# embedded-software-laboratory/p-dmpc

Hardware: AMD Instinct MI355X
Metric: MPC steps/sec (whole node) + p50 per-step plan latency, N vehicles H=8 (higher is better)
Workload: dtype f64

## Files before the change

include/pdmpc.h:

```cpp
#ifndef PDMPC_H
#define PDMPC_H

#include <stddef.h>
#include <stdint.h>

#ifdef __cplusplus
extern "C" {
#endif

#define PDMPC_HP_MAX 16
#define PDMPC_VMAX 8
#define PDMPC_JOINT_MAX 4

enum {
    PDMPC_OK = 0,
    PDMPC_EXHAUSTED = 1,
    PDMPC_ARENA_OVERFLOW = 2,
    PDMPC_ERR_INVALID = -1,
    PDMPC_ERR_NO_DEVICE = -2,
    PDMPC_ERR_HIP = -3,
    PDMPC_ERR_CAPACITY = -4,
    PDMPC_ERR_NO_MPA = -5
};

// ... 54 lines not shown
    const double* right_y;
    pdmpc_polygon_set obstacles;
    pdmpc_polygon_set dynamic_obstacles;
    pdmpc_polygon_set hdv_reachable_sets;
} pdmpc_vehicle_in;

typedef struct {
    int32_t status;
    int32_t n_expanded;
    int32_t n_popped;
    int32_t n_hp;
    int32_t tree_path[PDMPC_HP_MAX + 1];
    int32_t predicted_trims[PDMPC_HP_MAX];
    int32_t shape_cols[PDMPC_HP_MAX];
    int32_t _pad;
    double y_predicted[PDMPC_HP_MAX][3];
    double shapes[PDMPC_HP_MAX][2][PDMPC_VMAX];
    double path_nodes[PDMPC_HP_MAX + 1][8];
} pdmpc_vehicle_out;

typedef struct {
    int64_t n_vehicles;
    int64_t nodes_popped;
    int64_t nodes_generated;
    int64_t obstacle_columns;
    int64_t algorithmic_bytes;
    double kernel_ms;
    int64_t lds_bytes;
    int64_t lds_nodes;
    int64_t n_launches;
    int64_t queue_fallbacks;
    int64_t speculation_arrivals;
    int64_t edge_checks;
    int64_t segment_pair_tests;
    int64_t kernel;
    int64_t nodes_processed;
    int64_t rounds;
    int64_t shared_rounds;
    int64_t helper_checked;
    int64_t safe_replans;
    int64_t bad_status_plans;
} pdmpc_stats;


int pdmpc_create(const pdmpc_config* config, pdmpc_handle** out_handle);
int pdmpc_destroy(pdmpc_handle* handle);

int pdmpc_get_config(pdmpc_handle* handle, pdmpc_config* config, int32_t* mpa_uploaded);

int pdmpc_upload_mpa(pdmpc_handle* handle, const pdmpc_mpa* mpa);
int pdmpc_mpa_reach_host(const pdmpc_mpa* mpa, double* dmax, double* amax);
int pdmpc_reach_lists_host(int32_t Hp, double dmax, double amax, double root_x, double root_y, const double* x, const double* y, const int32_t* step_first,
                           const int32_t* step_count, int32_t* list_offset, int32_t* list);

int pdmpc_plan_batch(pdmpc_handle* handle, int32_t n_vehicles, const pdmpc_vehicle_in* in,
                     pdmpc_vehicle_out* out);

int pdmpc_set_arena_limit(pdmpc_handle* handle, int32_t max_nodes_limit);
int pdmpc_grow_arena(pdmpc_handle* handle, int32_t max_nodes);
int pdmpc_arena_nodes(pdmpc_handle* handle, int32_t* max_nodes, int64_t* regrows);

int pdmpc_plan_step(pdmpc_handle* handle, int32_t n_vehicles, const pdmpc_vehicle_in* in, const int32_t* pred_offset,
                    const int32_t* pred_index, const pdmpc_polygon_set* fallback_shapes, pdmpc_vehicle_out* out);

int pdmpc_plan_step_literal(pdmpc_handle* handle, int32_t n_vehicles, const pdmpc_vehicle_in* in, const int32_t* pred_offset, const int32_t* pred_index,
                            const pdmpc_polygon_set* fallback_shapes, pdmpc_vehicle_out* out);

int pdmpc_pack_batch(pdmpc_handle* handle, int32_t n_vehicles, const pdmpc_vehicle_in* in);
int pdmpc_plan_step_lean(pdmpc_handle* handle, int32_t n_vehicles, const pdmpc_vehicle_in* in, const int32_t* pred_offset, const int32_t* pred_index,
                         const pdmpc_polygon_set* fallback_shapes, int32_t* status, double* final_cost);
int pdmpc_fetch_records_at(pdmpc_handle* handle, int32_t count, const int32_t* vehicles, pdmpc_vehicle_out* out);
typedef struct {
    int32_t n_cells;
    int32_t n_graphs;
    int32_t n_picks;
    int32_t _pad;
    const int32_t* cell_offset;
    const int32_t* cell_slot;
    const int32_t* graph_offset;
    const int32_t* pick_graph;
    const int32_t* pick_offset;
    const int32_t* pick_slot;
} pdmpc_choice;
int pdmpc_choose_host(int32_t n, const int32_t* status, const double* final_cost, const pdmpc_choice* choice, int32_t* chosen, double* cell_cost);
int pdmpc_choose_resident(pdmpc_handle* handle, int32_t n, const pdmpc_choice* choice, int32_t* chosen, double* cell_cost, pdmpc_vehicle_out* picks);
int pdmpc_plan_step_chosen(pdmpc_handle* handle, int32_t n_vehicles, const pdmpc_vehicle_in* in, const int32_t* pred_offset, const int32_t* pred_index,
                           const pdmpc_polygon_set* fallback_shapes, const pdmpc_choice* choice, int32_t* chosen, double* cell_cost, pdmpc_vehicle_out* picks);
int pdmpc_choice_kernel_ms(pdmpc_handle* handle, double* ms);
int pdmpc_last_call_timing(pdmpc_handle* handle, double* us3);
int pdmpc_launch_packed(pdmpc_handle* handle);
int pdmpc_launch_range(pdmpc_handle* handle, int32_t first, int32_t count);
int pdmpc_fetch_results(pdmpc_handle* handle, int32_t n_vehicles, pdmpc_vehicle_out* out);
int pdmpc_synchronize(pdmpc_handle* handle);
int pdmpc_set_safe_launch(pdmpc_handle* handle, int32_t on);
int pdmpc_set_device_share(pdmpc_handle* handle, int32_t n_handles);
int pdmpc_begin_step(pdmpc_handle* handle);
int pdmpc_select_bank(pdmpc_handle* handle, int32_t bank);
int pdmpc_reset_stats(pdmpc_handle* handle);

int pdmpc_set_step_weights(pdmpc_handle* handle, int32_t n_vehicles, const double* weights);
int pdmpc_pack_step(pdmpc_handle* handle, int32_t n_vehicles, const pdmpc_vehicle_in* in,
                    const int32_t* pred_offset, const int32_t* pred_index,
                    const pdmpc_polygon_set* fallback_shapes);

int pdmpc_result_device_buffer(pdmpc_handle* handle, void** dev_ptr, size_t* nbytes);
int pdmpc_import_results(pdmpc_handle* handle, int32_t first, int32_t n, const void* dev_records);
// ... 223 lines not shown
```

include/pdmpc_reach.h:

```cpp
#ifndef PDMPC_REACH_H
#define PDMPC_REACH_H

#include <math.h>

#include "pdmpc_math.h"

#define PDMPC_REACH_FINITE 0x1p64
#define PDMPC_REACH_MARGIN 0x1p-20

PDMPC_HD static inline double pdmpc_reach_radius(double dmax, double amax, int k) {
    const double r = (double)(k - 1) * dmax + amax;
    return r + r * 0x1p-50;
}

PDMPC_HD static inline void pdmpc_reach_box(double dmax, double amax, int k, double root_x, double root_y, double* box) {
    const double R = pdmpc_reach_radius(dmax, amax, k);
    const double rho = R + PDMPC_REACH_MARGIN * (1.0 + fabs(root_x) + fabs(root_y) + R);
    box[0] = root_x - rho;
    box[1] = root_x + rho;
    box[2] = root_y - rho;
    box[3] = root_y + rho;
}

PDMPC_HD static inline int pdmpc_reach_in(double x0, double y0, double x1, double y1, double x_lo, double x_hi, double y_lo, double y_hi) {
    if (x0 != x0 || y0 != y0 || x1 != x1 || y1 != y1) return 0;
    const int bounded = fabs(x0) <= PDMPC_REACH_FINITE && fabs(y0) <= PDMPC_REACH_FINITE && fabs(x1) <= PDMPC_REACH_FINITE && fabs(y1) <= PDMPC_REACH_FINITE;
    if (!bounded) return 1;
    const double max_x = x0 > x1 ? x0 : x1, min_x = x0 < x1 ? x0 : x1;
    const double max_y = y0 > y1 ? y0 : y1, min_y = y0 < y1 ? y0 : y1;
    return !(max_x < x_lo || min_x > x_hi || max_y < y_lo || min_y > y_hi);
}

#endif
```

p-dmpc_amd/csrc/api.cpp:

```cpp
#include <hip/hip_runtime.h>

#include <algorithm>
#include <cmath>
#include <cstdio>
#include <cstdlib>
#include <chrono>
#include <cstring>
#include <limits>
#include <map>
#include <mutex>
#include <string>
#include <utility>
#include <vector>

#include "../../include/pdmpc_geometry.h"
#include "../../include/pdmpc_reach.h"
#include "handle.hpp"

namespace {

thread_local std::string g_err;

inline uint32_t align16(uint32_t v) { return (v + 15u) & ~15u; }

// ... 446 lines not shown
    }
    (void)hipMemsetAsync(h->d_flag.p, 0, h->d_flag.cap * sizeof(uint32_t), h->stream);
    (void)hipMemsetAsync(h->d_tree_size.p, 0, h->d_tree_size.cap * sizeof(int32_t), h->stream);
    (void)hipMemsetAsync(h->d_tie_count.p, 0, 4 * sizeof(int32_t), h->stream);
    (void)hipMemsetAsync(h->d_work_count.p, 0, 16 * sizeof(unsigned long long), h->stream);
    (void)hipMemsetAsync(h->d_out.p, 0, h->d_out.cap * sizeof(pdmpc_vehicle_out), h->stream);
    (void)hipStreamSynchronize(h->stream);
    *out_handle = h;
    return PDMPC_OK;
}

int pdmpc_destroy(pdmpc_handle* h) {
    if (!h) return PDMPC_OK;
    DeviceGuard device_guard__(h->cfg.device);
    delete h;
    return PDMPC_OK;
}

static void mpa_reach(const pdmpc_mpa* mpa, double& dmax, double& amax) {
    dmax = 0.0;
    amax = 0.0;
    for (int t = 0; t < mpa->n_maneuvers; ++t) {
        const pdmpc_maneuver& m = mpa->maneuvers[t];
        dmax = std::max(dmax, hypot(m.dx, m.dy));
        const double(*src[3])[PDMPC_VMAX] = {m.area, m.area_without_offset, m.area_large_offset};
        for (int a = 0; a < 3; ++a)
            for (int v = 0; v < m.n_cols && v < PDMPC_VMAX; ++v) amax = std::max(amax, hypot(src[a][0][v], src[a][1][v]));
    }
}

int pdmpc_mpa_reach_host(const pdmpc_mpa* mpa, double* dmax, double* amax) {
    if (!mpa || !dmax || !amax || (mpa->n_maneuvers > 0 && !mpa->maneuvers)) return fail(PDMPC_ERR_INVALID, "pdmpc_mpa_reach_host: null argument");
    mpa_reach(mpa, *dmax, *amax);
    return PDMPC_OK;
}

int pdmpc_reach_lists_host(int32_t Hp, double dmax, double amax, double root_x, double root_y, const double* x, const double* y, const int32_t* step_first,
                           const int32_t* step_count, int32_t* list_offset, int32_t* list) {
    if (Hp < 1 || Hp > PDMPC_HP_MAX || !step_first || !step_count || !list_offset) return fail(PDMPC_ERR_INVALID, "pdmpc_reach_lists_host: bad argument");
    int32_t n = 0;
    for (int k = 1; k <= Hp; ++k) {
        const int32_t a = step_first[k - 1], c = step_count[k - 1];
        if (a < 0 || c < 0 || (c > 1 && (!x || !y || !list))) return fail(PDMPC_ERR_INVALID, "pdmpc_reach_lists_host: bad step ranges");
        double box[4];
        pdmpc_reach_box(dmax, amax, k, root_x, root_y, box);
        list_offset[k - 1] = n;
        for (int32_t j = 0; j + 1 < c; ++j)
            if (pdmpc_reach_in(x[a + j], y[a + j], x[a + j + 1], y[a + j + 1], box[0], box[1], box[2], box[3])) list[n++] = j;
    }
    list_offset[Hp] = n;
    return PDMPC_OK;
}

int pdmpc_upload_mpa(pdmpc_handle* h, const pdmpc_mpa* mpa) {
    if (!h || !mpa) return fail(PDMPC_ERR_INVALID, "null argument");
    if (mpa->n_trims < 1 || mpa->n_trims > 1023) return fail(PDMPC_ERR_INVALID, "n_trims must be in 1..1023");
    if (mpa->Hp < h->cfg.Hp) return fail(PDMPC_ERR_INVALID, "mpa.Hp smaller than config.Hp");
    if (!mpa->transition || !mpa->maneuver_index || (mpa->n_maneuvers > 0 && !mpa->maneuvers)) return fail(PDMPC_ERR_INVALID, "null table");
    ON_DEVICE(h->cfg.device);
    const int n = mpa->n_trims, Hp = h->cfg.Hp;
    const int nw = (n + 63) / 64;
    std::vector<uint64_t> mask((size_t)Hp * n * nw + 2, 0);
    for (int k = 0; k < Hp; ++k)
        for (int i = 0; i < n; ++i)
            for (int j = 0; j < n; ++j)
                if (mpa->transition[((size_t)k * n + i) * n + j]) {
                    const int mi = mpa->maneuver_index[i * n + j];
                    if (mi < 0 || mi >= mpa->n_maneuvers) return fail(PDMPC_ERR_INVALID, "transition allowed but maneuver missing");
                    mask[((size_t)k * n + i) * nw + j / 64] |= 1ull << (j % 64);
                }
    std::vector<int16_t> mi((size_t)n * n + 8, -1);
    for (int i = 0; i < n * n; ++i) mi[i] = (int16_t)mpa->maneuver_index[i];
    const int T = mpa->n_maneuvers;
    std::vector<DevManPose> pose((size_t)std::max(T, 1));
    std::vector<double> area((size_t)std::max(T, 1) * 3 * PDMPC_VMAX * 2 + 2, 0.0);
    for (int t = 0; t < T; ++t) {
        const pdmpc_maneuver& m = mpa->maneuvers[t];
        if (m.n_cols < 2 || m.n_cols > PDMPC_VMAX) return fail(PDMPC_ERR_INVALID, "maneuver area column count out of range");
        pose[t].dx = m.dx;
        pose[t].dy = m.dy;
        pose[t].dyaw = m.dyaw;
        pose[t].n_cols = m.n_cols;
        pose[t].pad = 0;
        const double(*src[3])[PDMPC_VMAX] = {m.area, m.area_without_offset, m.area_large_offset};
        for (int a = 0; a < 3; ++a)
            for (int v = 0; v < m.n_cols; ++v) {
                area[(((size_t)t * 3 + a) * PDMPC_VMAX + v) * 2 + 0] = src[a][0][v];
                area[(((size_t)t * 3 + a) * PDMPC_VMAX + v) * 2 + 1] = src[a][1][v];
            }
    }
    mpa_reach(mpa, area[(size_t)T * 3 * PDMPC_VMAX * 2], area[(size_t)T * 3 * PDMPC_VMAX * 2 + 1]);
    if (h->d_mask.ensure(mask.size()) || h->d_mi.ensure(mi.size()) || h->d_pose.ensure(pose.size()) || h->d_area.ensure(area.size()))
        return fail(PDMPC_ERR_HIP, "hipMalloc failed for the MPA tables");
    HIPCHK(hipMemcpy(h->d_mask.p, mask.data(), mask.size() * 8, hipMemcpyHostToDevice));
    HIPCHK(hipMemcpy(h->d_mi.p, mi.data(), mi.size() * 2, hipMemcpyHostToDevice));
    HIPCHK(hipMemcpy(h->d_pose.p, pose.data(), pose.size() * sizeof(DevManPose), hipMemcpyHostToDevice));
    HIPCHK(hipMemcpy(h->d_area.p, area.data(), area.size() * 8, hipMemcpyHostToDevice));
    h->n_trims = n;
    h->n_words = nw;
    h->n_man = T;
    h->mask_bytes = (size_t)Hp * n * nw * 8;
    h->mi_bytes = (size_t)n * n * 2;
    h->mpa_alg_bytes = (int64_t)8 * T * (3 + 6 * PDMPC_VMAX) + (int64_t)n * n * Hp / 8;
    h->has_mpa = true;
    return PDMPC_OK;
}

int pdmpc_pack_batch(pdmpc_handle* h, int32_t n, const pdmpc_vehicle_in* in) { return pdmpc_pack_step(h, n, in, nullptr, nullptr, nullptr); }

int pdmpc_pack_step(pdmpc_handle* h, int32_t n, const pdmpc_vehicle_in* in, const int32_t* pred_offset, const int32_t* pred_index,
                    const pdmpc_polygon_set* fallback_shapes) {
    if (!h) return fail(PDMPC_ERR_INVALID, "null handle");
    ON_DEVICE(h->cfg.device);
    if (pred_offset && !pred_index) return fail(PDMPC_ERR_INVALID, "pred_index missing");
    return pack_common(h, n, in, pred_offset, pred_index, fallback_shapes);
}

int pdmpc_set_step_weights(pdmpc_handle* h, int32_t n, const double* weights) {
    if (!h || n < 0 || (n > 0 && !weights)) return fail(PDMPC_ERR_INVALID, "pdmpc_set_step_weights: bad argument");
    h->next_weights.assign(weights, weights + n);
    return PDMPC_OK;
}

int pdmpc_set_step_seeds(pdmpc_handle* h, int32_t n, const uint32_t* seeds) {
    if (!h || n < 0 || (n > 0 && !seeds)) return fail(PDMPC_ERR_INVALID, "pdmpc_set_step_seeds: bad argument");
    h->next_seeds.assign(seeds, seeds + n);
    h->seeds_set = true;
    return PDMPC_OK;
}

int pdmpc_launch_packed(pdmpc_handle* h) {
    if (!h) return fail(PDMPC_ERR_INVALID, "null handle");
    ON_DEVICE(h->cfg.device);
    h->epoch += 1;
    return launch_range(h, 0, h->banks[h->bank].n_packed, h->safe_launches);
}

int pdmpc_set_device_share(pdmpc_handle* h, int32_t n_handles) {
    if (!h || n_handles < 1) return fail(PDMPC_ERR_INVALID, "pdmpc_set_device_share: bad argument");
    h->device_share = n_handles;
    return PDMPC_OK;
}

int pdmpc_set_safe_launch(pdmpc_handle* h, int32_t on) {
// ... 953 lines not shown
```

p-dmpc_amd/csrc/bulk_search.hpp:

```cpp
#include <hip/hip_runtime.h>

#include "search_common.hpp"

#include "frontier_common.hpp"

#include "../../include/pdmpc_reach.h"

#define BK_P2 3
#define BK_PER PDMPC_BK_PER
#define BK_FAST_PER 4

namespace {

typedef volatile LDS_AS unsigned long long lds_vu64;
typedef LDS_AS uint16_t lds_u16;

__device__ __forceinline__ unsigned long long wg_scan_excl(unsigned long long v, lds_vu64* wsum, int lane, int wave, int n_waves, unsigned long long& total) {
    unsigned long long inc = v;
#pragma unroll
    for (int o = 1; o < PDMPC_WAVE; o <<= 1) {
        const unsigned long long t = __shfl_up(inc, o);
        inc += lane >= o ? t : 0ull;
    }
    if (lane == PDMPC_WAVE - 1) wsum[wave] = inc;
    __syncthreads();
    unsigned long long off = 0, tot = 0;
    for (int q = 0; q < n_waves; ++q) {
        const unsigned long long w = wsum[q];
        off += q < wave ? w : 0ull;
        tot += w;
    }
    total = tot;
    return off + inc - v;
}

__device__ __forceinline__ d2 node_piece(const Search& S, uint32_t i0, int q) {
    if (i0 < S.NL) return S.ln[4 * (size_t)i0 + q];
    return ((const d2*)(S.gn + i0))[q];
}
__device__ __forceinline__ void piece_link(d2 p3, uint32_t& parent, uint32_t& packed) {
    const uint64_t u = (uint64_t)__double_as_longlong(p3.y);
    parent = (uint32_t)(u & 0xffffffffull);
    packed = (uint32_t)(u >> 32);
}

struct BkCheck {
    const lds_d2* l_area;
    const d2* g_area;
    const lds_d2* l_soup;
    const lds_i32* l_soff;
    const lds_i32* l_hoff;
    const lds_i32* l_lit;
    int areas_in_lds, ll_base, ll_len, Hp;
};

#define BK_RLIST(lsm) ((lds_u16*)((lsm) + PDMPC_LK_FIXED_END))
__device__ __forceinline__ LDS_AS unsigned char* bk_lds_base() {
    extern __shared__ __attribute__((aligned(16))) unsigned char smem[];
    return (LDS_AS unsigned char*)smem;
}
#define BK_RBOX(lsm) ((lds_f64*)((lsm) + PDMPC_LK_REACH))
#define BK_RCNT(lsm) ((lds_u32*)((lsm) + PDMPC_LK_REACH + PDMPC_LK_REACH_CNT))
#define BK_RSTALE(lsm) ((volatile lds_u32*)((lsm) + PDMPC_LK_REACH + PDMPC_LK_REACH_STALE))
#define BK_RSC(lsm) ((lds_i32*)((lsm) + PDMPC_LK_REACH + PDMPC_LK_REACH_SC))
__device__ __forceinline__ void bk_reach_scalars(const BkCheck& C, LDS_AS unsigned char* lsm, bool shared_boundary_list) {
    lds_i32* sc = BK_RSC(lsm);
    sc[0] = (int32_t)((LDS_AS unsigned char*)C.l_soup - lsm);
    sc[1] = (int32_t)((LDS_AS unsigned char*)C.l_area - lsm);
    sc[2] = C.Hp;
    sc[3] = C.ll_base;
    sc[4] = C.ll_len;
    sc[5] = shared_boundary_list ? 0 : C.ll_len;
}
struct BkItemCtx {
    const BkCheck& C;
    int interx;
    __device__ __forceinline__ int word(int i) const { return BK_RSC(bk_lds_base())[i]; }
    __device__ __forceinline__ const lds_d2* l_soup() const { return interx ? (const lds_d2*)(bk_lds_base() + word(0)) : C.l_soup; }
    __device__ __forceinline__ const lds_d2* l_area() const { return interx ? (const lds_d2*)(bk_lds_base() + word(1)) : C.l_area; }
    __device__ __forceinline__ int Hp() const { return interx ? word(2) : C.Hp; }
    __device__ __forceinline__ int ll_base() const { return interx ? word(3) : C.ll_base; }
    __device__ __forceinline__ int ll_stride() const { return interx ? word(5) : C.ll_len; }
};
template <int CHECKER>
__device__ __forceinline__ BkItemCtx bk_item_ctx(const BkCheck& C) {
    return BkItemCtx{C, CHECKER == PDMPC_CHECK_INTERX ? 1 : 0};
}
__device__ __forceinline__ void bk_reach_boxes(const KernelArgs& A, const DevVehicle* V, LDS_AS unsigned char* lsm, int tid) {
    if (tid < A.Hp) {
        const double* reach = A.man_area + (size_t)A.n_man * 3 * PDMPC_VMAX * 2;
        double box[4];
        pdmpc_reach_box(reach[0], reach[1], tid + 1, V->x0, V->y0, box);
        lds_f64* rb = BK_RBOX(lsm) + 4 * tid;
        rb[0] = box[0];
        rb[1] = box[1];
        rb[2] = box[2];
        rb[3] = box[3];
    }
}
template <int SOUPS>
__device__ __forceinline__ void bk_reach_build(const BkCheck& C, LDS_AS unsigned char* lsm, int lane, int wave, int n_waves) {
    const lds_f64* rbox = BK_RBOX(lsm);
    lds_u32* rcnt = BK_RCNT(lsm);
    for (int u = wave; u < (SOUPS == 1 ? 1 : 3) * C.Hp; u += n_waves) {
        const int k = SOUPS == 1 ? u : u / 3, s = SOUPS == 1 ? 0 : u - 3 * k;
        int base, n, at, kb = k;
        if (s == 0) {
            base = C.l_soff[k];
            n = C.l_soff[k + 1] - base - 1;
            at = base;
        } else if (s == 1) {
            base = C.l_hoff[k];
            n = C.l_hoff[k + 1] - base - 1;
            at = base;
        } else {
            const int stride = BK_RSC(lsm)[5];
            base = C.ll_base;
            n = C.ll_len - 1;
            at = base + k * stride;
            kb = stride ? k : C.Hp - 1;
        }
        const double x_lo = rbox[4 * kb], x_hi = rbox[4 * kb + 1], y_lo = rbox[4 * kb + 2], y_hi = rbox[4 * kb + 3];
        const lds_d2* q = C.l_soup + base;
        lds_u16* lst = BK_RLIST(lsm) + at;
        uint32_t cnt = 0;
        for (int j0 = 0; j0 < n; j0 += PDMPC_WAVE) {
            const int j = j0 + lane;
            bool in = false;
            if (j < n) {
                const d2 q0 = q[j], q1 = q[j + 1];
                in = pdmpc_reach_in(q0.x, q0.y, q1.x, q1.y, x_lo, x_hi, y_lo, y_hi) != 0;
            }
            const unsigned long long m = __ballot(in);
            if (in) lst[cnt + __builtin_amdgcn_mbcnt_hi((uint32_t)(m >> 32), __builtin_amdgcn_mbcnt_lo((uint32_t)m, 0u))] = (uint16_t)j;
            cnt += (uint32_t)__builtin_popcountll(m);
        }
        if (lane == 0) rcnt[s * PDMPC_HP_MAX + k] = cnt;
    }
}

#define VS_TENT 6u

__device__ __forceinline__ void bk_tentative_areas(const KernelArgs& A, const SpecCtx& P, unsigned long long who, int tid, int nthreads) {
    const double qnan = __longlong_as_double(0x7ff8000000000000LL);
    const int per = P.Hp * PDMPC_VMAX, n_pred = P.n_pred < 64 ? P.n_pred : 64;
    for (int idx = tid; idx < n_pred * per; idx += nthreads) {
        const int p = idx / per, rest = idx - p * per;
        if (!((who >> p) & 1ull)) continue;
        const DevVehicle* PV = A.veh + P.pred[p];
        if (PV->fb_off[0] < 0) continue;
        const int k = rest / PDMPC_VMAX, v = rest - k * PDMPC_VMAX;
        const int a = PV->fb_off[k], b = PV->fb_off[k + 1];
        const int cols = (b - a < PDMPC_VMAX) ? (b - a) : PDMPC_VMAX;
        d2 pt;
        pt.x = v < cols ? A.points[2 * (size_t)(a + (v < cols ? v : 0))] : qnan;
        pt.y = v < cols ? A.points[2 * (size_t)(a + (v < cols ? v : 0)) + 1] : qnan;
        P.l_soup[P.l_soff[k] + P.l_lit[k] + p * PDMPC_VMAX + v] = pt;
    }
}

struct BkTreeSrc {
    const Search* S;
    const lds_u32* ready;
    __device__ __forceinline__ void link(uint32_t r, uint32_t& parent, uint32_t& packed) const { piece_link(node_piece(*S, ready[r] - 1u, 3), parent, packed); }
    __device__ __forceinline__ void pose(uint32_t, uint32_t parent, double& px, double& py, double& cs, double& sn) const {
        const d2 pxy = node_piece(*S, parent - 1u, 0), pcs = node_piece(*S, parent - 1u, 2);
        px = pxy.x;
        py = pxy.y;
        cs = pcs.x;
        sn = pcs.y;
    }
};
struct BkPostSrc {
    const lds_d2* rec;
    __device__ __forceinline__ void link(uint32_t r, uint32_t& parent, uint32_t& packed) const { piece_link(d2{0.0, rec[3 * r + 2].x}, parent, packed); }
    __device__ __forceinline__ void pose(uint32_t r, uint32_t, double& px, double& py, double& cs, double& sn) const {
        const d2 pxy = rec[3 * r], pcs = rec[3 * r + 1];
        px = pxy.x;
        py = pxy.y;
        cs = pcs.x;
        sn = pcs.y;
    }
};

// ... 351 lines not shown
__device__ __forceinline__ void bk_publish_flag(const KernelArgs& A, int slot, int lane) {
    asm volatile("s_waitcnt vmcnt(0)" ::: "memory");
    wave_sync();
    if (lane == 0) {
        __hip_atomic_store(A.done_flag + slot, A.epoch, __ATOMIC_RELAXED, __HIP_MEMORY_SCOPE_AGENT);
    }
}
__device__ __forceinline__ void bk_publish(const KernelArgs& A, const Ctx& X, int status, bool dep_timeout) {
    if (X.lane == 0 && (dep_timeout || (status != PDMPC_OK && status != PDMPC_EXHAUSTED))) atomicAdd(A.work_count + 6, 1ull);
    bk_publish_flag(A, X.slot, X.lane);
}

__device__ __forceinline__ unsigned long long bk_poll_flags(const KernelArgs& A, const SpecCtx& P, unsigned long long want, int lane) {
    bool d = false;
    if ((want >> lane) & 1ull) d = __hip_atomic_load(A.done_flag + P.pred[lane], __ATOMIC_RELAXED, __HIP_MEMORY_SCOPE_AGENT) == A.epoch;
    const unsigned long long got = __ballot(d);
    return got;
}

__device__ __forceinline__ bool bk_poll_predecessors(const KernelArgs& A, const SpecCtx& P, volatile lds_u32* sh, unsigned long long skip, int lane) {
    const unsigned long long pend = sh_load64(sh, SH_PEND_LO) & ~skip;
    if (!pend) return false;
    const unsigned long long got = bk_poll_flags(A, P, pend, lane);
    if (!got) return false;
    if (lane == 0) {
        sh[SH_ARR_LO] = (uint32_t)got;
        sh[SH_ARR_HI] = (uint32_t)(got >> 32);
        __builtin_amdgcn_fence(__ATOMIC_RELEASE, "workgroup");
        atomicCAS((uint32_t*)&sh[SH_STATE], ST_RUN, ST_ARRIVED);
    }
    return true;
}

__device__ __forceinline__ void bk_incorporate_body(const pdmpc_vehicle_out* out, const int32_t* pred, lds_d2* l_soup, const lds_i32* l_soff, const lds_i32* l_lit, int Hp, unsigned long long arr, int tid,
                                                    int nthreads, lds_u64s* chg, const lds_f64* rbox) {
    const double qnan = __longlong_as_double(0x7ff8000000000000LL);
    const int per = Hp * PDMPC_VMAX, n_arr = __builtin_popcountll(arr);
    for (int idx = tid; idx < n_arr * per; idx += nthreads) {
        const int a = idx / per, rest = idx - a * per;
        const int p = nth_bit(arr, a);
        const pdmpc_vehicle_out* PO = out + pred[p];
        const int k = rest / PDMPC_VMAX, v = rest - k * PDMPC_VMAX;
        const int cols = bk_area_load_i32(&PO->shape_cols[k]);
        const double sx = bk_area_load(&PO->shapes[k][0][v]), sy = bk_area_load(&PO->shapes[k][1][v]);
        d2 pt;
        pt.x = v < cols ? sx : qnan;
        pt.y = v < cols ? sy : qnan;
        lds_d2* slot = l_soup + l_soff[k] + l_lit[k] + p * PDMPC_VMAX + v;
        if (chg) {
            const d2 was = *slot;
            const bool differs = __double_as_longlong(was.x) != __double_as_longlong(pt.x) || __double_as_longlong(was.y) != __double_as_longlong(pt.y);
            if (rbox) {
                const double nx = __shfl_down(pt.x, 1), ny = __shfl_down(pt.y, 1);
                const bool in = v + 1 < PDMPC_VMAX && pdmpc_reach_in(pt.x, pt.y, nx, ny, rbox[4 * k], rbox[4 * k + 1], rbox[4 * k + 2], rbox[4 * k + 3]) != 0;
                const int g = (tid & (PDMPC_WAVE - 1)) & ~(PDMPC_VMAX - 1);
                const unsigned long long md = __ballot(differs), mi = __ballot(in);
                if (v == 0 && ((md >> g) & 0xffull) != 0ull && ((mi >> g) & 0xffull) != 0ull)
                    __hip_atomic_fetch_or(chg + k, 1ull << p, __ATOMIC_RELAXED, __HIP_MEMORY_SCOPE_WORKGROUP);
            } else if (differs) {
                __hip_atomic_fetch_or(chg + k, 1ull << p, __ATOMIC_RELAXED, __HIP_MEMORY_SCOPE_WORKGROUP);
            }
        }
        *slot = pt;
    }
}
__device__ __forceinline__ void bk_incorporate(const pdmpc_vehicle_out* out, const int32_t* pred, lds_d2* l_soup, const lds_i32* l_soff, const lds_i32* l_lit, int Hp, unsigned long long arr, int tid,
                                               int nthreads, lds_u64s* chg, const lds_f64* rbox) {
    bk_incorporate_body(out, pred, l_soup, l_soff, l_lit, Hp, arr, tid, nthreads, chg, rbox);
}

#define WC_DEAD 0x100u
#define WC_ONPATH 0x200u
#define WC_VALID 0x400u
__device__ int bk_classify_wave(const unsigned long long* glink, ulonglong2* walk, const VState& VS, const double* gkey, const lds_u32* gp_path, const lds_f64* gp_mp, bool have_goal,
                                bool check_alive, uint32_t best, uint32_t epoch, uint32_t a, double ka, volatile lds_u32* sh) {
    const uint32_t a0 = a ? a : 1u;
    const uint64_t ua = glink[a0 - 1u];
    const uint32_t p = (uint32_t)(ua & 0xffffffffull);
    const int k = NODE_K((uint32_t)(ua >> 32));
    const bool onp = have_goal && gp_path[k] == a0;
    const ulonglong2 c = walk[p ? p - 1u : 0u];
    const uint32_t ctag = (uint32_t)(c.y & 0xffffffffull), cinfo = (uint32_t)(c.y >> 32);
    const bool hit = p != 0u && ctag == best && (cinfo & (WC_VALID | 0xffff0000u)) == (WC_VALID | (epoch << 16));
    double M = -1.0;
    int dJ = k;
    bool dead = false;
    int st = (a == 0u || onp || hit) ? 1 : 0;
    uint32_t x = a0;
    while (__ballot(st == 0)) {
        const uint32_t i = x - 1u;
        const uint64_t u = glink[i];
        const int d = NODE_K((uint32_t)(u >> 32));
        const bool on_path = have_goal && gp_path[d] == x;
        const bool bad = !on_path && x != a0 && check_alive && vs_load(VS, i) != VS_VALID;
        const double kx = gkey[i];
        const uint32_t par = (uint32_t)(u & 0xffffffffull);
        const bool walking = st == 0;
        const bool stop = on_path || bad || par == 0u;
        dJ = (walking && on_path) ? d : dJ;
        dead = dead || (walking && bad);
        M = (walking && !on_path && !bad && kx > M) ? kx : M;
        st = (walking && stop) ? 1 : st;
        x = (walking && !stop) ? par : x;
    }
    if (hit && !onp) {
        const bool p_on = (cinfo & WC_ONPATH) != 0u;
        const double pM = __longlong_as_double((long long)c.x);
// ... 1872 lines not shown
```

p-dmpc_amd/csrc/pdmpc_device.h:

```cpp
#ifndef PDMPC_DEVICE_H
#define PDMPC_DEVICE_H

#include <stdint.h>

#include "../../include/pdmpc.h"

#define PDMPC_WAVE 64
#define PDMPC_MAX_WAVES 16
#define PDMPC_MAX_WAVES_SAT 12
#define PDMPC_SH_WORDS 128

struct DevManPose {
    double dx, dy, dyaw;
    int32_t n_cols;
    int32_t pad;
};

struct DevVehicle {
    double x0, y0, yaw0;
    double ref_x[PDMPC_HP_MAX];
    double ref_y[PDMPC_HP_MAX];
    double v_ref[PDMPC_HP_MAX];
    int32_t trim0;
    int32_t n_pred;
// ... 25 lines not shown
    uint32_t soup;
    uint32_t cand;
    uint32_t vstate;
    uint32_t expand;
    uint32_t tree16;
    uint32_t rand;
    uint32_t nodes;
    uint32_t total;
    uint32_t bk_near_key, bk_near_id;
    uint32_t bk_ready;
    uint32_t bk_hist;
    uint32_t bk_misc;
    uint32_t bk_pshape;
    uint32_t reach_shared;
    uint32_t bk_reach;
    uint32_t reach;
};

struct LdsPathRegion {
    uint32_t path[PDMPC_HP_MAX + 2];
    int32_t soff[PDMPC_HP_MAX + 1];
    int32_t hoff[PDMPC_HP_MAX + 1];
    uint32_t shared[PDMPC_SH_WORDS];
    int32_t lit[PDMPC_HP_MAX];
};
#define PDMPC_LK_PATH_BYTES PDMPC_LK_ALIGN16((uint32_t)sizeof(LdsPathRegion))

#define PDMPC_LK_ALIGN16(x) (((x) + 15u) & ~15u)
#ifndef PDMPC_LK_WAVES
#define PDMPC_LK_WAVES PDMPC_MAX_WAVES
#endif
#ifndef PDMPC_LK_READY_CAP
#define PDMPC_LK_READY_CAP 2048u
#endif
#define PDMPC_LK_COMPACT_WAVES 8
#define PDMPC_LK_COMPACT_READY_CAP 512u
#define PDMPC_LK_COMPACT_BK_PER 2
#define PDMPC_LKX_THREADS(W) ((uint32_t)(W) * PDMPC_WAVE)
#define PDMPC_LKX_REF 0u
#define PDMPC_LKX_SHAPE (PDMPC_LKX_REF + 3u * PDMPC_HP_MAX * 8u)
#define PDMPC_LKX_PATH(W) (PDMPC_LKX_SHAPE + (uint32_t)(W) * (2u * PDMPC_VMAX + 1u) * 16u)
#define PDMPC_LKX_CAND(W) (PDMPC_LKX_PATH(W) + PDMPC_LK_PATH_BYTES)
#define PDMPC_LKX_EXPAND(W) (PDMPC_LKX_CAND(W) + PDMPC_LK_ALIGN16(12u * PDMPC_LKX_THREADS(W)))
#define PDMPC_LKX_NEAR_KEY(W) (PDMPC_LKX_EXPAND(W) + (2u * PDMPC_HP_MAX * PDMPC_HP_MAX) * 8u + 16u * 16u)
#define PDMPC_LKX_NEAR_ID(W, P) (PDMPC_LKX_NEAR_KEY(W) + PDMPC_LK_ALIGN16((uint32_t)(P) * PDMPC_LKX_THREADS(W) * 8u))
#define PDMPC_LKX_READY(W, P) (PDMPC_LKX_NEAR_ID(W, P) + PDMPC_LK_ALIGN16((uint32_t)(P) * PDMPC_LKX_THREADS(W) * 4u))
#define PDMPC_LKX_HIST(W, RC, P) (PDMPC_LKX_READY(W, P) + (uint32_t)(RC) * 8u)
#define PDMPC_LKX_MISC(W, RC, P) (PDMPC_LKX_HIST(W, RC, P) + 3072u * 4u)
#define PDMPC_LKX_PSHAPE(W, RC, P) (PDMPC_LKX_MISC(W, RC, P) + 2048u)
#define PDMPC_LKX_REACH(W, RC, P) (PDMPC_LKX_PSHAPE(W, RC, P) + PDMPC_LK_ALIGN16(PDMPC_HP_MAX * PDMPC_VMAX * 16u + PDMPC_HP_MAX * 4u + PDMPC_HP_MAX * 8u + PDMPC_HP_MAX * 4u))
#define PDMPC_LK_REACH_CNT (PDMPC_HP_MAX * 4u * 8u)
#define PDMPC_LK_REACH_STALE (PDMPC_LK_REACH_CNT + 3u * PDMPC_HP_MAX * 4u)
#define PDMPC_LK_REACH_SC (PDMPC_LK_REACH_STALE + 16u)
#define PDMPC_LKX_FIXED_END(W, RC, P) (PDMPC_LKX_REACH(W, RC, P) + PDMPC_LK_REACH_SC + 32u)
#ifndef PDMPC_BK_PER
#define PDMPC_BK_PER 4
#endif
#define PDMPC_LK_REF PDMPC_LKX_REF
#define PDMPC_LK_SHAPE PDMPC_LKX_SHAPE
#define PDMPC_LK_PATH PDMPC_LKX_PATH(PDMPC_LK_WAVES)
#define PDMPC_LK_CAND PDMPC_LKX_CAND(PDMPC_LK_WAVES)
#define PDMPC_LK_EXPAND PDMPC_LKX_EXPAND(PDMPC_LK_WAVES)
#define PDMPC_LK_NEAR_KEY PDMPC_LKX_NEAR_KEY(PDMPC_LK_WAVES)
#define PDMPC_LK_NEAR_ID PDMPC_LKX_NEAR_ID(PDMPC_LK_WAVES, PDMPC_BK_PER)
#define PDMPC_LK_READY PDMPC_LKX_READY(PDMPC_LK_WAVES, PDMPC_BK_PER)
#define PDMPC_LK_HIST PDMPC_LKX_HIST(PDMPC_LK_WAVES, PDMPC_LK_READY_CAP, PDMPC_BK_PER)
#define PDMPC_LK_MISC PDMPC_LKX_MISC(PDMPC_LK_WAVES, PDMPC_LK_READY_CAP, PDMPC_BK_PER)
#define PDMPC_LK_PSHAPE PDMPC_LKX_PSHAPE(PDMPC_LK_WAVES, PDMPC_LK_READY_CAP, PDMPC_BK_PER)
#define PDMPC_LK_REACH PDMPC_LKX_REACH(PDMPC_LK_WAVES, PDMPC_LK_READY_CAP, PDMPC_BK_PER)
#define PDMPC_LK_FIXED_END PDMPC_LKX_FIXED_END(PDMPC_LK_WAVES, PDMPC_LK_READY_CAP, PDMPC_BK_PER)

struct NodeArena {
    NodeRec* nodes;
    double* key;
    unsigned long long* link;
    uint8_t* vstate;
    double* far_key;
    uint32_t* far_id;
    double* mid_key;
    uint32_t* mid_id;
    double* pb_key;
    uint32_t* pb_d;
    double* walk;
    uint32_t* child0;
    uint32_t* vlist;
};

static inline uint32_t pdmpc_lk_fixed(uint32_t W, uint32_t RC, uint32_t P, LdsLayout* L) {
    L->ref = PDMPC_LKX_REF;
    L->shape = PDMPC_LKX_SHAPE;
    L->path = PDMPC_LKX_PATH(W);
    L->cand = PDMPC_LKX_CAND(W);
    L->expand = PDMPC_LKX_EXPAND(W);
    L->bk_near_key = PDMPC_LKX_NEAR_KEY(W);
    L->bk_near_id = PDMPC_LKX_NEAR_ID(W, P);
    L->bk_ready = PDMPC_LKX_READY(W, P);
    L->bk_hist = PDMPC_LKX_HIST(W, RC, P);
    L->bk_misc = PDMPC_LKX_MISC(W, RC, P);
    L->bk_pshape = PDMPC_LKX_PSHAPE(W, RC, P);
    L->bk_reach = PDMPC_LKX_REACH(W, RC, P);
    return PDMPC_LKX_FIXED_END(W, RC, P);
}

#define PDMPC_HELP_CAP 2048
#define PDMPC_HB_SEATS_MAX 64
#define PDMPC_HB_N 1
#define PDMPC_HB_MASK 2
// ... 278 lines not shown
```

p-dmpc_amd/pdmpc/prototypes.py:

```python
import ctypes as C

from . import abi

P = C.POINTER
INT, STR = C.c_int, C.c_char_p
OBJ = C.c_void_p
VOIDP = C.c_void_p
I32, I64, U32, F64 = C.c_int32, C.c_int64, C.c_uint32, C.c_double
DP, IP, BP, UP = abi.c_double_p, abi.c_int32_p, abi.c_uint8_p, abi.c_uint32_p
CONFIG, MPA, POLYS, VIN, VOUT, CHOICE = P(abi.Config), P(abi.Mpa), P(abi.PolygonSet), P(abi.VehicleIn), P(abi.VehicleOut), P(abi.ChoiceStruct)

STEP = [I32, VIN, IP, IP, POLYS]
STEP_OUT = [P(I32), P(VIN), P(IP), P(IP), P(POLYS)]
POSES = [DP, DP, DP, DP, IP]
TABLE = [I32, I32, POLYS]
COUPLED = [BP, DP]
BOUND = POSES + [POLYS, I32, I32, IP, DP, DP, BP]
FCA = [I32, I32, DP, DP, DP, DP, I32, IP, POLYS, POLYS, F64, F64, F64, IP, IP]
FCA_GROUPED = [I32, P(abi.FcaGroup), I32, DP, DP, DP, DP, IP, IP]
CHOSEN = [CHOICE, IP, DP]
UNIQUE = [I32, BP, I64, P(I64), UP, IP]
UNIQUE_GROUPED = [I32, IP, P(BP), P(I64), P(I64), UP, IP]

PROTOTYPES = {
    "pdmpc_create": (INT, [CONFIG, P(OBJ)]),
    "pdmpc_destroy": (INT, [OBJ]),
    "pdmpc_get_config": (INT, [OBJ, CONFIG, P(I32)]),
    "pdmpc_upload_mpa": (INT, [OBJ, MPA]),
    "pdmpc_mpa_reach_host": (INT, [MPA, DP, DP]),
    "pdmpc_reach_lists_host": (INT, [I32, F64, F64, F64, F64, DP, DP, IP, IP, IP, IP]),
    "pdmpc_plan_batch": (INT, [OBJ, I32, VIN, VOUT]),
    "pdmpc_set_arena_limit": (INT, [OBJ, I32]),
    "pdmpc_grow_arena": (INT, [OBJ, I32]),
    "pdmpc_arena_nodes": (INT, [OBJ, P(I32), P(I64)]),
    "pdmpc_plan_step": (INT, [OBJ] + STEP + [VOUT]),
    "pdmpc_plan_step_literal": (INT, [OBJ] + STEP + [VOUT]),
    "pdmpc_pack_batch": (INT, [OBJ, I32, VIN]),
    "pdmpc_plan_step_lean": (INT, [OBJ] + STEP + [IP, DP]),
    "pdmpc_fetch_records_at": (INT, [OBJ, I32, IP, VOUT]),
    "pdmpc_choose_host": (INT, [I32, IP, DP] + CHOSEN),
    "pdmpc_choose_resident": (INT, [OBJ, I32] + CHOSEN + [VOUT]),
    "pdmpc_plan_step_chosen": (INT, [OBJ] + STEP + CHOSEN + [VOUT]),
    "pdmpc_choice_kernel_ms": (INT, [OBJ, DP]),
    "pdmpc_last_call_timing": (INT, [OBJ, DP]),
    "pdmpc_launch_packed": (INT, [OBJ]),
    "pdmpc_launch_range": (INT, [OBJ, I32, I32]),
    "pdmpc_fetch_results": (INT, [OBJ, I32, VOUT]),
    "pdmpc_synchronize": (INT, [OBJ]),
    "pdmpc_set_safe_launch": (INT, [OBJ, I32]),
    "pdmpc_set_device_share": (INT, [OBJ, I32]),
    "pdmpc_begin_step": (INT, [OBJ]),
    "pdmpc_select_bank": (INT, [OBJ, I32]),
    "pdmpc_reset_stats": (INT, [OBJ]),
    "pdmpc_set_step_weights": (INT, [OBJ, I32, DP]),
    "pdmpc_pack_step": (INT, [OBJ] + STEP),
    "pdmpc_result_device_buffer": (INT, [OBJ, P(VOIDP), P(C.c_size_t)]),
    "pdmpc_import_results": (INT, [OBJ, I32, I32, VOIDP]),
    "pdmpc_export_results": (INT, [OBJ, I32, I32, VOIDP]),
    "pdmpc_export_results_async": (INT, [OBJ, I32, I32, VOIDP]),
    "pdmpc_stream": (INT, [OBJ, P(VOIDP)]),
    "pdmpc_get_last_stats": (INT, [OBJ, P(abi.Stats)]),
    "pdmpc_debug_pop_trace": (INT, [OBJ, I32, I32, IP, IP]),
    "pdmpc_debug_tree": (INT, [OBJ, I32, I32] + [DP] * 5 + [IP] * 4),
    "pdmpc_debug_edge_check": (INT, [OBJ, I32, I32, IP, DP, DP, IP, DP, DP, IP]),
    "pdmpc_debug_raw_tree": (INT, [OBJ, I32, I32] + [DP] * 5 + [IP] * 3 + [DP, BP, IP]),
    "pdmpc_debug_counters": (INT, [OBJ, P(C.c_uint64)]),
    "pdmpc_debug_progress": (INT, [OBJ, I32, UP]),
    "pdmpc_debug_heap_script": (INT, [OBJ, I32, IP, IP, DP, I32, IP, IP, DP, DP]),
    "pdmpc_plan_batch_sampled": (INT, [OBJ, I32, VIN, UP, VOUT]),
    "pdmpc_plan_step_sampled": (INT, [OBJ] + STEP + [UP, VOUT]),
    "pdmpc_set_step_seeds": (INT, [OBJ, I32, UP]),
    "pdmpc_debug_random_numbers": (INT, [OBJ, I32, UP, I32, DP]),
    "pdmpc_plan_joint": (INT, [OBJ, I32, IP, VIN, VOUT]),
    "pdmpc_unique_priorities": (INT, [OBJ] + UNIQUE),
    "pdmpc_unique_priorities_host": (INT, UNIQUE),
    "pdmpc_unique_priorities_grouped": (INT, [OBJ] + UNIQUE_GROUPED),
    "pdmpc_unique_priorities_grouped_host": (INT, UNIQUE_GROUPED),
    "pdmpc_local_reachable_sets": (INT, [MPA, I32, IP, DP, DP]),
    "pdmpc_upload_reachable_sets": (INT, [OBJ] + TABLE),
    "pdmpc_reachable_set_coupling": (INT, [OBJ, I32] + POSES + COUPLED),
    "pdmpc_reachable_set_coupling_host": (INT, TABLE + [I32] + POSES + COUPLED),
    "pdmpc_reachable_set_coupling_kernel_ms": (INT, [OBJ, DP]),
    "pdmpc_bound_reachable_sets": (INT, [OBJ, I32] + BOUND),
# ... 90 lines not shown
```

Before: 1572.

## Tighten reachability culling with per-trim oriented reach rectangles from MPA hulls

Replaces the isotropic radius-based reach box with per-trim, per-step rectangles in the vehicle frame. They are precomputed at MPA upload from convex hulls of composed maneuver areas. Device culling now rotates boundary segments into the root frame before testing them, so fewer boundary segments should enter the collision lists and later checks do less work. In exchange, each segment test costs more arithmetic, upload does extra hull work, and LDS use grows slightly.

```diff
diff --git a/include/pdmpc.h b/include/pdmpc.h
--- a/include/pdmpc.h
+++ b/include/pdmpc.h
@@ -130,6 +130,9 @@
 int pdmpc_mpa_reach_host(const pdmpc_mpa* mpa, double* dmax, double* amax);
 int pdmpc_reach_lists_host(int32_t Hp, double dmax, double amax, double root_x, double root_y, const double* x, const double* y, const int32_t* step_first,
                            const int32_t* step_count, int32_t* list_offset, int32_t* list);
+int pdmpc_mpa_reach_rects_host(const pdmpc_mpa* mpa, int32_t Hp, double* rects);
+int pdmpc_reach_lists_oriented_host(int32_t Hp, int32_t n_trims, const double* rects, int32_t root_trim, double root_x, double root_y, double root_yaw, const double* x, const double* y,
+                                    const int32_t* step_first, const int32_t* step_count, int32_t* list_offset, int32_t* list);
 
 int pdmpc_plan_batch(pdmpc_handle* handle, int32_t n_vehicles, const pdmpc_vehicle_in* in,
                      pdmpc_vehicle_out* out);
diff --git a/include/pdmpc_reach.h b/include/pdmpc_reach.h
--- a/include/pdmpc_reach.h
+++ b/include/pdmpc_reach.h
@@ -31,4 +31,30 @@
     return !(max_x < x_lo || min_x > x_hi || max_y < y_lo || min_y > y_hi);
 }
 
+#define PDMPC_REACH_ROTATION 0x1p-48
+
+PDMPC_HD static inline void pdmpc_reach_rect_box(const double* rect, double root_x, double root_y, double* box) {
+    const double ax = fabs(rect[0]) > fabs(rect[1]) ? fabs(rect[0]) : fabs(rect[1]);
+    const double ay = fabs(rect[2]) > fabs(rect[3]) ? fabs(rect[2]) : fabs(rect[3]);
+    const double m = PDMPC_REACH_MARGIN * (1.0 + fabs(root_x) + fabs(root_y) + (ax > ay ? ax : ay));
+    box[0] = rect[0] - m;
+    box[1] = rect[1] + m;
+    box[2] = rect[2] - m;
+    box[3] = rect[3] + m;
+}
+
+PDMPC_HD static inline int pdmpc_reach_in_oriented(double x0, double y0, double x1, double y1, double root_x, double root_y, double cs, double sn, double x_lo, double x_hi, double y_lo,
+                                                   double y_hi) {
+    if (x0 != x0 || y0 != y0 || x1 != x1 || y1 != y1) return 0;
+    const int bounded = fabs(x0) <= PDMPC_REACH_FINITE && fabs(y0) <= PDMPC_REACH_FINITE && fabs(x1) <= PDMPC_REACH_FINITE && fabs(y1) <= PDMPC_REACH_FINITE;
+    if (!bounded) return 1;
+    const double dx0 = x0 - root_x, dy0 = y0 - root_y, dx1 = x1 - root_x, dy1 = y1 - root_y;
+    const double u0 = cs * dx0 + sn * dy0, v0 = cs * dy0 - sn * dx0;
+    const double u1 = cs * dx1 + sn * dy1, v1 = cs * dy1 - sn * dx1;
+    const double slack = PDMPC_REACH_ROTATION * (fabs(dx0) + fabs(dy0) + fabs(dx1) + fabs(dy1));
+    const double max_u = u0 > u1 ? u0 : u1, min_u = u0 < u1 ? u0 : u1;
+    const double max_v = v0 > v1 ? v0 : v1, min_v = v0 < v1 ? v0 : v1;
+    return !(max_u < x_lo - slack || min_u > x_hi + slack || max_v < y_lo - slack || min_v > y_hi + slack);
+}
+
 #endif
diff --git a/p-dmpc_amd/csrc/api.cpp b/p-dmpc_amd/csrc/api.cpp
--- a/p-dmpc_amd/csrc/api.cpp
+++ b/p-dmpc_amd/csrc/api.cpp
@@ -522,6 +522,121 @@
     return PDMPC_OK;
 }
 
+namespace {
+typedef std::pair<double, double> ReachPt;
+void reach_hull(std::vector<ReachPt>& P, std::vector<ReachPt>& H) {
+    std::sort(P.begin(), P.end());
+    P.erase(std::unique(P.begin(), P.end()), P.end());
+    const size_t n = P.size();
+    if (n < 3) return;
+    auto cross = [](const ReachPt& o, const ReachPt& a, const ReachPt& b) { return (a.first - o.first) * (b.second - o.second) - (a.second - o.second) * (b.first - o.first); };
+    H.clear();
+    for (size_t i = 0; i < n; ++i) {
+        while (H.size() >= 2 && cross(H[H.size() - 2], H.back(), P[i]) <= 0) H.pop_back();
+        H.push_back(P[i]);
+    }
+    const size_t lower = H.size() + 1;
+    for (size_t i = n - 1; i-- > 0;) {
+        while (H.size() >= lower && cross(H[H.size() - 2], H.back(), P[i]) <= 0) H.pop_back();
+        H.push_back(P[i]);
+    }
+    H.pop_back();
+    P.swap(H);
+}
+void mpa_reach_rects(const pdmpc_mpa* mpa, int Hp, double* rects) {
+    const int n = mpa->n_trims, T = mpa->n_maneuvers;
+    const double qnan = std::numeric_limits<double>::quiet_NaN();
+    std::vector<double> cs((size_t)std::max(T, 1)), sn((size_t)std::max(T, 1));
+    for (int t = 0; t < T; ++t) pdmpc_sincos(mpa->maneuvers[t].dyaw, &sn[t], &cs[t]);
+    auto maneuver = [&](int k, int i, int j) {
+        if (!mpa->transition[((size_t)(k - 1) * n + i) * n + j]) return -1;
+        const int t = mpa->maneuver_index[(size_t)i * n + j];
+        return t >= 0 && t < T ? t : -1;
+    };
+    std::vector<int> slice((size_t)Hp);
+    for (int k = 0; k < Hp; ++k) {
+        slice[k] = k;
+        for (int q = 0; q < k; ++q)
+            if (!memcmp(mpa->transition + (size_t)q * n * n, mpa->transition + (size_t)k * n * n, (size_t)n * n)) {
+                slice[k] = slice[q];
+                break;
+            }
+    }
+    typedef std::vector<std::vector<ReachPt>> Table;
+    std::map<std::vector<int>, size_t> known;
+    std::vector<Table> tables;
+    std::vector<ReachPt> scratch;
+    for (int K = 1; K <= Hp; ++K) {
+        size_t at = 0;
+        for (int k = K; k >= 1; --k) {
+            const std::vector<int> key(slice.begin() + (k - 1), slice.begin() + K);
+            const auto found = known.find(key);
+            if (found != known.end()) {
+                at = found->second;
+                continue;
+            }
+            Table t((size_t)n);
+            for (int i = 0; i < n; ++i) {
+                for (int j = 0; j < n; ++j) {
+                    const int mi = maneuver(k, i, j);
+                    if (mi < 0) continue;
+                    const pdmpc_maneuver& m = mpa->maneuvers[mi];
+                    if (k == K) {
+                        const double(*src[3])[PDMPC_VMAX] = {m.area, m.area_without_offset, m.area_large_offset};
+                        for (int a = 0; a < 3; ++a)
+                            for (int v = 0; v < m.n_cols && v < PDMPC_VMAX; ++v) t[i].push_back(ReachPt(src[a][0][v], src[a][1][v]));
+                    } else {
+                        for (const ReachPt& p : tables[at][j]) t[i].push_back(ReachPt(cs[mi] * p.first - sn[mi] * p.second + m.dx, sn[mi] * p.first + cs[mi] * p.second + m.dy));
+                    }
+                }
+                reach_hull(t[i], scratch);
+            }
+            at = tables.size();
+            tables.push_back(std::move(t));
+            known[key] = at;
+        }
+        const Table& cur = tables[at];
+        for (int i = 0; i < n; ++i) {
+            double* r = rects + ((size_t)i * Hp + (K - 1)) * 4;
+            r[0] = r[1] = r[2] = r[3] = qnan;
+            for (const ReachPt& p : cur[i]) {
+                r[0] = p.first < r[0] || r[0] != r[0] ? p.first : r[0];
+                r[1] = p.first > r[1] || r[1] != r[1] ? p.first : r[1];
+                r[2] = p.second < r[2] || r[2] != r[2] ? p.second : r[2];
+                r[3] = p.second > r[3] || r[3] != r[3] ? p.second : r[3];
+            }
+        }
+    }
+}
+}
+
+int pdmpc_mpa_reach_rects_host(const pdmpc_mpa* mpa, int32_t Hp, double* rects) {
+    if (!mpa || !rects || !mpa->transition || !mpa->maneuver_index || (mpa->n_maneuvers > 0 && !mpa->maneuvers)) return fail(PDMPC_ERR_INVALID, "pdmpc_mpa_reach_rects_host: null argument");
+    if (mpa->n_trims < 1 || Hp < 1 || Hp > PDMPC_HP_MAX || Hp > mpa->Hp) return fail(PDMPC_ERR_INVALID, "pdmpc_mpa_reach_rects_host: Hp out of range");
+    mpa_reach_rects(mpa, Hp, rects);
+    return PDMPC_OK;
+}
+
+int pdmpc_reach_lists_oriented_host(int32_t Hp, int32_t n_trims, const double* rects, int32_t root_trim, double root_x, double root_y, double root_yaw, const double* x, const double* y,
+                                    const int32_t* step_first, const int32_t* step_count, int32_t* list_offset, int32_t* list) {
+    if (Hp < 1 || Hp > PDMPC_HP_MAX || !rects || root_trim < 1 || root_trim > n_trims || !step_first || !step_count || !list_offset)
+        return fail(PDMPC_ERR_INVALID, "pdmpc_reach_lists_oriented_host: bad argument");
+    double cs, sn;
+    pdmpc_sincos(root_yaw, &sn, &cs);
+    int32_t n = 0;
+    for (int k = 1; k <= Hp; ++k) {
+        const int32_t a = step_first[k - 1], c = step_count[k - 1];
+        if (a < 0 || c < 0 || (c > 1 && (!x || !y || !list))) return fail(PDMPC_ERR_INVALID, "pdmpc_reach_lists_oriented_host: bad step ranges");
+        double box[4];
+        pdmpc_reach_rect_box(rects + ((size_t)(root_trim - 1) * Hp + (k - 1)) * 4, root_x, root_y, box);
+        list_offset[k - 1] = n;
+        for (int32_t j = 0; j + 1 < c; ++j)
+            if (pdmpc_reach_in_oriented(x[a + j], y[a + j], x[a + j + 1], y[a + j + 1], root_x, root_y, cs, sn, box[0], box[1], box[2], box[3])) list[n++] = j;
+    }
+    list_offset[Hp] = n;
+    return PDMPC_OK;
+}
+
 int pdmpc_upload_mpa(pdmpc_handle* h, const pdmpc_mpa* mpa) {
     if (!h || !mpa) return fail(PDMPC_ERR_INVALID, "null argument");
     if (mpa->n_trims < 1 || mpa->n_trims > 1023) return fail(PDMPC_ERR_INVALID, "n_trims must be in 1..1023");
@@ -543,7 +658,7 @@
     for (int i = 0; i < n * n; ++i) mi[i] = (int16_t)mpa->maneuver_index[i];
     const int T = mpa->n_maneuvers;
     std::vector<DevManPose> pose((size_t)std::max(T, 1));
-    std::vector<double> area((size_t)std::max(T, 1) * 3 * PDMPC_VMAX * 2 + 2, 0.0);
+    std::vector<double> area((size_t)std::max(T, 1) * 3 * PDMPC_VMAX * 2 + 2 + (size_t)n * Hp * 4, 0.0);
     for (int t = 0; t < T; ++t) {
         const pdmpc_maneuver& m = mpa->maneuvers[t];
         if (m.n_cols < 2 || m.n_cols > PDMPC_VMAX) return fail(PDMPC_ERR_INVALID, "maneuver area column count out of range");
@@ -560,6 +675,7 @@
             }
     }
     mpa_reach(mpa, area[(size_t)T * 3 * PDMPC_VMAX * 2], area[(size_t)T * 3 * PDMPC_VMAX * 2 + 1]);
+    mpa_reach_rects(mpa, Hp, &area[(size_t)T * 3 * PDMPC_VMAX * 2 + 2]);
     if (h->d_mask.ensure(mask.size()) || h->d_mi.ensure(mi.size()) || h->d_pose.ensure(pose.size()) || h->d_area.ensure(area.size()))
         return fail(PDMPC_ERR_HIP, "hipMalloc failed for the MPA tables");
     HIPCHK(hipMemcpy(h->d_mask.p, mask.data(), mask.size() * 8, hipMemcpyHostToDevice));
diff --git a/p-dmpc_amd/csrc/bulk_search.hpp b/p-dmpc_amd/csrc/bulk_search.hpp
--- a/p-dmpc_amd/csrc/bulk_search.hpp
+++ b/p-dmpc_amd/csrc/bulk_search.hpp
@@ -63,6 +63,7 @@
 #define BK_RCNT(lsm) ((lds_u32*)((lsm) + PDMPC_LK_REACH + PDMPC_LK_REACH_CNT))
 #define BK_RSTALE(lsm) ((volatile lds_u32*)((lsm) + PDMPC_LK_REACH + PDMPC_LK_REACH_STALE))
 #define BK_RSC(lsm) ((lds_i32*)((lsm) + PDMPC_LK_REACH + PDMPC_LK_REACH_SC))
+#define BK_RROOT(lsm) ((lds_f64*)((lsm) + PDMPC_LK_REACH + PDMPC_LK_REACH_ROOT))
 __device__ __forceinline__ void bk_reach_scalars(const BkCheck& C, LDS_AS unsigned char* lsm, bool shared_boundary_list) {
     lds_i32* sc = BK_RSC(lsm);
     sc[0] = (int32_t)((LDS_AS unsigned char*)C.l_soup - lsm);
@@ -88,14 +89,40 @@
 }
 __device__ __forceinline__ void bk_reach_boxes(const KernelArgs& A, const DevVehicle* V, LDS_AS unsigned char* lsm, int tid) {
     if (tid < A.Hp) {
-        const double* reach = A.man_area + (size_t)A.n_man * 3 * PDMPC_VMAX * 2;
+        const int at = A.n_man * (3 * PDMPC_VMAX * 2) + 2 + ((V->trim0 - 1) * A.Hp + tid) * 4;
+        const double r[4] = {A.man_area[at], A.man_area[at + 1], A.man_area[at + 2], A.man_area[at + 3]};
         double box[4];
-        pdmpc_reach_box(reach[0], reach[1], tid + 1, V->x0, V->y0, box);
+        pdmpc_reach_rect_box(r, V->x0, V->y0, box);
         lds_f64* rb = BK_RBOX(lsm) + 4 * tid;
         rb[0] = box[0];
         rb[1] = box[1];
         rb[2] = box[2];
         rb[3] = box[3];
+    } else if (tid == A.Hp) {
+        double cs, sn;
+        pdmpc_sincos(V->yaw0, &sn, &cs);
+        lds_f64* rr = BK_RROOT(lsm);
+        rr[0] = V->x0;
+        rr[1] = V->y0;
+        rr[2] = cs;
+        rr[3] = sn;
+        if (A.lds.reach_shared != 0u) {
+            const double* rect = A.man_area + (A.n_man * (3 * PDMPC_VMAX * 2) + 2 + (V->trim0 - 1) * A.Hp * 4);
+            double lo_x = 0.0, hi_x = 0.0, lo_y = 0.0, hi_y = 0.0;
+            for (int k = 0; k < A.Hp; ++k) {
+                const double r[4] = {rect[4 * k], rect[4 * k + 1], rect[4 * k + 2], rect[4 * k + 3]};
+                double box[4];
+                pdmpc_reach_rect_box(r, V->x0, V->y0, box);
+                lo_x = k == 0 || !(box[0] >= lo_x) ? box[0] : lo_x;
+                hi_x = k == 0 || !(box[1] <= hi_x) ? box[1] : hi_x;
+                lo_y = k == 0 || !(box[2] >= lo_y) ? box[2] : lo_y;
+                hi_y = k == 0 || !(box[3] <= hi_y) ? box[3] : hi_y;
+            }
+            rr[4] = lo_x;
+            rr[5] = hi_x;
+            rr[6] = lo_y;
+            rr[7] = hi_y;
+        }
     }
 }
 template <int SOUPS>
@@ -105,6 +132,7 @@
     for (int u = wave; u < (SOUPS == 1 ? 1 : 3) * C.Hp; u += n_waves) {
         const int k = SOUPS == 1 ? u : u / 3, s = SOUPS == 1 ? 0 : u - 3 * k;
         int base, n, at, kb = k;
+        bool one_list = false;
         if (s == 0) {
             base = C.l_soff[k];
             n = C.l_soff[k + 1] - base - 1;
@@ -119,8 +147,10 @@
             n = C.ll_len - 1;
             at = base + k * stride;
             kb = stride ? k : C.Hp - 1;
-        }
-        const double x_lo = rbox[4 * kb], x_hi = rbox[4 * kb + 1], y_lo = rbox[4 * kb + 2], y_hi = rbox[4 * kb + 3];
+            one_list = stride == 0;
+        }
+        const lds_f64* rb = one_list ? BK_RROOT(lsm) + 4 : rbox + 4 * kb;
+        const lds_f64* root = BK_RROOT(lsm);
         const lds_d2* q = C.l_soup + base;
         lds_u16* lst = BK_RLIST(lsm) + at;
         uint32_t cnt = 0;
@@ -129,7 +159,7 @@
             bool in = false;
             if (j < n) {
                 const d2 q0 = q[j], q1 = q[j + 1];
-                in = pdmpc_reach_in(q0.x, q0.y, q1.x, q1.y, x_lo, x_hi, y_lo, y_hi) != 0;
+                in = pdmpc_reach_in_oriented(q0.x, q0.y, q1.x, q1.y, root[0], root[1], root[2], root[3], rb[0], rb[1], rb[2], rb[3]) != 0;
             }
             const unsigned long long m = __ballot(in);
             if (in) lst[cnt + __builtin_amdgcn_mbcnt_hi((uint32_t)(m >> 32), __builtin_amdgcn_mbcnt_lo((uint32_t)m, 0u))] = (uint16_t)j;
@@ -587,7 +617,8 @@
             const bool differs = __double_as_longlong(was.x) != __double_as_longlong(pt.x) || __double_as_longlong(was.y) != __double_as_longlong(pt.y);
             if (rbox) {
                 const double nx = __shfl_down(pt.x, 1), ny = __shfl_down(pt.y, 1);
-                const bool in = v + 1 < PDMPC_VMAX && pdmpc_reach_in(pt.x, pt.y, nx, ny, rbox[4 * k], rbox[4 * k + 1], rbox[4 * k + 2], rbox[4 * k + 3]) != 0;
+                const lds_f64* root = rbox + (PDMPC_LK_REACH_ROOT >> 3);
+                const bool in = v + 1 < PDMPC_VMAX && pdmpc_reach_in_oriented(pt.x, pt.y, nx, ny, root[0], root[1], root[2], root[3], rbox[4 * k], rbox[4 * k + 1], rbox[4 * k + 2], rbox[4 * k + 3]) != 0;
                 const int g = (tid & (PDMPC_WAVE - 1)) & ~(PDMPC_VMAX - 1);
                 const unsigned long long md = __ballot(differs), mi = __ballot(in);
                 if (v == 0 && ((md >> g) & 0xffull) != 0ull && ((mi >> g) & 0xffull) != 0ull)
diff --git a/p-dmpc_amd/csrc/pdmpc_device.h b/p-dmpc_amd/csrc/pdmpc_device.h
--- a/p-dmpc_amd/csrc/pdmpc_device.h
+++ b/p-dmpc_amd/csrc/pdmpc_device.h
@@ -101,7 +101,8 @@
 #define PDMPC_LK_REACH_CNT (PDMPC_HP_MAX * 4u * 8u)
 #define PDMPC_LK_REACH_STALE (PDMPC_LK_REACH_CNT + 3u * PDMPC_HP_MAX * 4u)
 #define PDMPC_LK_REACH_SC (PDMPC_LK_REACH_STALE + 16u)
-#define PDMPC_LKX_FIXED_END(W, RC, P) (PDMPC_LKX_REACH(W, RC, P) + PDMPC_LK_REACH_SC + 32u)
+#define PDMPC_LK_REACH_ROOT (PDMPC_LK_REACH_SC + 32u)
+#define PDMPC_LKX_FIXED_END(W, RC, P) (PDMPC_LKX_REACH(W, RC, P) + PDMPC_LK_REACH_ROOT + 64u)
 #ifndef PDMPC_BK_PER
 #define PDMPC_BK_PER 4
 #endif
diff --git a/p-dmpc_amd/pdmpc/prototypes.py b/p-dmpc_amd/pdmpc/prototypes.py
--- a/p-dmpc_amd/pdmpc/prototypes.py
+++ b/p-dmpc_amd/pdmpc/prototypes.py
@@ -29,6 +29,8 @@
     "pdmpc_upload_mpa": (INT, [OBJ, MPA]),
     "pdmpc_mpa_reach_host": (INT, [MPA, DP, DP]),
     "pdmpc_reach_lists_host": (INT, [I32, F64, F64, F64, F64, DP, DP, IP, IP, IP, IP]),
+    "pdmpc_mpa_reach_rects_host": (INT, [MPA, I32, DP]),
+    "pdmpc_reach_lists_oriented_host": (INT, [I32, I32, DP, I32, F64, F64, F64, DP, DP, IP, IP, IP, IP]),
     "pdmpc_plan_batch": (INT, [OBJ, I32, VIN, VOUT]),
     "pdmpc_set_arena_limit": (INT, [OBJ, I32]),
     "pdmpc_grow_arena": (INT, [OBJ, I32]),
```

After: 1614 (median of 6 runs). 2.7% higher.
